# ChristophReich1996/Semantic_Pyramid_for_Image_Generation

Measured on AMD Instinct MI355X. Metric: images/sec full G+D train step, 256x256, bs/GPU=20, higher is better.
Workload: dtype bf16

## Files before the change

### include/sempyr.h

```cpp
#ifndef SEMPYR_H
#define SEMPYR_H
#include <stdint.h>

#ifdef __cplusplus
extern "C" {
#endif

#define SP_VERSION 1

typedef void* sp_stream_t;

enum sp_status { SP_OK = 0, SP_ERR_INVALID = -1, SP_ERR_LAUNCH = -2, SP_ERR_UNSUPPORTED = -3 };
enum sp_dtype { SP_F32 = 0, SP_BF16 = 1, SP_F8 = 2 ,
                SP_F16 = 3 ,
                SP_F8_F16 = 4  };
enum sp_act { SP_ACT_NONE = 0, SP_ACT_LRELU = 1, SP_ACT_RELU = 2, SP_ACT_TANH = 3 };

int sp_version(void);

enum { SP_TUNE_CONV_TALL = 0, SP_TUNE_IGEMM_DMA = 1, SP_TUNE_WGRAD_ROWS = 2, SP_TUNE_DETERMINISTIC = 3,
       SP_TUNE_SPLITK_TARGET = 4, SP_TUNE_SPLITK_MINSTEPS = 5, SP_TUNE_CONV1X1_DIRECT = 6, SP_TUNE_CONV_SHORT = 7,
       SP_TUNE_WGRAD9_BLOCKS = 8, SP_TUNE_WGRAD_BLOCKS = 9, SP_TUNE_WGRAD_MINSTEPS = 10, SP_TUNE_WGRAD_SMALL_M = 11,
       SP_TUNE_WGRAD_K1_TILE64 = 12, SP_TUNE_WGRAD_ROWS_THIN = 13, SP_TUNE_WGRAD_ROWS_BLOCKS = 14, SP_TUNE_WGRAD_ROWS_SLABS = 15,
       SP_TUNE_CONV_STAGGER = 16, SP_TUNE_CONV1X1_SPLITK = 17, SP_TUNE_WGRAD1X1 = 18, SP_TUNE_CONV_CIN8 = 19, SP_TUNE_CONV_THINCO = 20, SP_TUNE_CONV_PP = 21, SP_TUNE_CONV_PP_PRIO = 22, SP_TUNE_WGRAD_PP = 23, SP_TUNE_BN_ITERS = 24, SP_TUNE_IGEMM_TILE = 25, SP_TUNE_CONV_PPW = 26, SP_TUNE_LINEAR_KS = 27, SP_TUNE_CONV_PP_SPLIT = 28, SP_TUNE_COUNT = 29 };
int sp_set_tuning(int32_t key, int32_t value);
const char* sp_last_error_string(void);
const char* sp_last_route(void);

typedef struct sp_conv_params {
    const void* x;
    const void* w;
    const float* bias;
    void* y;
    const void* res1;
    const void* res2;
    const void* mask_src;
    float mask_neg_slope;
    int32_t n, h, w_, cin_p, cout, ldy, ksize, act, dtype;
    void* workspace;
    int64_t workspace_bytes;
    int32_t pool2;
    int32_t in_up2;
    const float* x_scale;
    const float* w_scale;
    void* y8;
    const float* y8_inv_scale;
    float* y8_amax;
    const float* img_scale;
    int32_t img_split;
    int32_t reserved_;
    int64_t split_pix_;
    const void* tail_w;
    const float* tail_bias;
    void* tail_y;
    int32_t tail_cout, tail_act, tail_ld, reserved2_;
    uint32_t* pool_idx;
    int32_t* split_sync;
} sp_conv_params;
#define SP_CONV_SPLIT_SYNC_BYTES 8192
int sp_conv2d_igemm(const sp_conv_params* p, sp_stream_t stream);
int sp_conv2d_workspace(int32_t n, int32_t h, int32_t w_, int32_t cin_p, int32_t cout, int32_t ksize, int32_t dtype,
                        int64_t* bytes_out);
int sp_conv2d_route(const sp_conv_params* p, const char** route);

int sp_conv2d_wgrad(const void* x, const void* dy, float* dw, int32_t n, int32_t h, int32_t w_,
                    int32_t cin_p, int32_t cout, int32_t ld_dy, int32_t ksize, int32_t dtype,
                    sp_stream_t stream);

int sp_conv2d_wgrad_fused(const void* x, const void* dy, float* dw, float* dbias, const void* w_packed, float* dot,
                          float* workspace, int64_t workspace_floats, int32_t n, int32_t h, int32_t w_, int32_t cin_p,
                          int32_t cout, int32_t ld_dy, int32_t ksize, int32_t dtype, sp_stream_t stream);
int sp_conv2d_wgrad_accum(const void* x, const void* dy, float* dw, float* dbias, float* workspace, int64_t workspace_floats,
                          int32_t n, int32_t h, int32_t w_, int32_t cin_p, int32_t cout, int32_t ld_dy, int32_t ksize,
                          int32_t dtype, sp_stream_t stream);
int sp_conv2d_wgrad_accum_pooled(const void* x, const void* dy, float* dw, float* dbias, float* workspace, int64_t workspace_floats,
                                 int32_t n, int32_t h, int32_t w_, int32_t cin_p, int32_t cout, int32_t ld_dy, int32_t ksize,
                                 int32_t dtype, sp_stream_t stream);
// ... 227 lines not shown
```

### semantic_pyramid_for_image_generation_amd/_lib.py

```python
from __future__ import annotations

import ctypes
import os
import re
from typing import Dict, List, Tuple

_HERE = os.path.dirname(os.path.abspath(__file__))
HEADER = os.path.join(os.path.dirname(_HERE), "include", "sempyr.h")
LIB_PATH = os.environ.get("SEMPYR_LIB") or os.path.join(_HERE, "libsempyr.so")

SP_F32, SP_BF16, SP_F8, SP_F16, SP_F8_F16 = 0, 1, 2, 3, 4
ACT_NONE, ACT_LRELU, ACT_RELU, ACT_TANH = 0, 1, 2, 3

TUNE_KEYS = {"SP_CONV_TALL": 0, "SP_IGEMM_DMA": 1, "SP_WGRAD_ROWS": 2, "SP_DETERMINISTIC": 3, "SP_SPLITK_TARGET": 4,
             "SP_SPLITK_MINSTEPS": 5, "SP_CONV1X1_DIRECT": 6, "SP_CONV_SHORT": 7, "SP_WGRAD9_BLOCKS": 8, "SP_WGRAD_BLOCKS": 9,
             "SP_WGRAD_MINSTEPS": 10, "SP_WGRAD_SMALL_M": 11, "SP_WGRAD_K1_TILE64": 12, "SP_WGRAD_ROWS_THIN": 13,
             "SP_WGRAD_ROWS_BLOCKS": 14, "SP_WGRAD_ROWS_SLABS": 15, "SP_CONV_STAGGER": 16, "SP_CONV1X1_SPLITK": 17, "SP_WGRAD1X1": 18, "SP_CONV_CIN8": 19, "SP_CONV_THINCO": 20,
             "SP_CONV_PP": 21, "SP_CONV_PP_PRIO": 22, "SP_WGRAD_PP": 23, "SP_BN_ITERS": 24, "SP_IGEMM_TILE": 25, "SP_CONV_PPW": 26, "SP_LINEAR_KS": 27, "SP_CONV_PP_SPLIT": 28}


SP_CONV_SPLIT_SYNC_BYTES = 8192


class SpConvParams(ctypes.Structure):
    _fields_ = [("x", ctypes.c_void_p), ("w", ctypes.c_void_p), ("bias", ctypes.c_void_p), ("y", ctypes.c_void_p),
                ("res1", ctypes.c_void_p), ("res2", ctypes.c_void_p), ("mask_src", ctypes.c_void_p),
                ("mask_neg_slope", ctypes.c_float),
                ("n", ctypes.c_int32), ("h", ctypes.c_int32), ("w_", ctypes.c_int32), ("cin_p", ctypes.c_int32),
                ("cout", ctypes.c_int32), ("ldy", ctypes.c_int32), ("ksize", ctypes.c_int32), ("act", ctypes.c_int32),
                ("dtype", ctypes.c_int32), ("workspace", ctypes.c_void_p), ("workspace_bytes", ctypes.c_int64),
                ("pool2", ctypes.c_int32), ("in_up2", ctypes.c_int32),
                ("x_scale", ctypes.c_void_p), ("w_scale", ctypes.c_void_p), ("y8", ctypes.c_void_p),
                ("y8_inv_scale", ctypes.c_void_p), ("y8_amax", ctypes.c_void_p),
                ("img_scale", ctypes.c_void_p), ("img_split", ctypes.c_int32), ("reserved_", ctypes.c_int32),
                ("split_pix_", ctypes.c_int64),
                ("tail_w", ctypes.c_void_p), ("tail_bias", ctypes.c_void_p), ("tail_y", ctypes.c_void_p),
                ("tail_cout", ctypes.c_int32), ("tail_act", ctypes.c_int32), ("tail_ld", ctypes.c_int32), ("reserved2_", ctypes.c_int32),
                ("pool_idx", ctypes.c_void_p), ("split_sync", ctypes.c_void_p)]


class SpConvGeneralParams(ctypes.Structure):
    _fields_ = [("struct_bytes", ctypes.c_int32), ("dtype", ctypes.c_int32),
                ("x", ctypes.c_void_p), ("w", ctypes.c_void_p), ("bias", ctypes.c_void_p), ("y", ctypes.c_void_p),
                ("n", ctypes.c_int32), ("h", ctypes.c_int32), ("w_", ctypes.c_int32), ("cin_p", ctypes.c_int32),
                ("ldx", ctypes.c_int32), ("cout", ctypes.c_int32), ("ldy", ctypes.c_int32), ("kh", ctypes.c_int32),
                ("kw", ctypes.c_int32), ("stride_h", ctypes.c_int32), ("stride_w", ctypes.c_int32), ("pad_h", ctypes.c_int32),
                ("pad_w", ctypes.c_int32), ("act", ctypes.c_int32)]

    def __init__(self, **kw):
        super().__init__(struct_bytes=ctypes.sizeof(SpConvGeneralParams), **kw)


class SpSnLayer(ctypes.Structure):
    _fields_ = [("w", ctypes.c_void_p), ("u", ctypes.c_void_p), ("v", ctypes.c_void_p),
                ("scratch_off", ctypes.c_int64), ("part_off", ctypes.c_int64), ("fwd_off", ctypes.c_int64),
                ("dgrad_off", ctypes.c_int64),
                ("rows", ctypes.c_int32), ("cols", ctypes.c_int32), ("cin", ctypes.c_int32), ("taps", ctypes.c_int32),
                ("cin_p", ctypes.c_int32), ("cout_p", ctypes.c_int32), ("kind", ctypes.c_int32),
                ("pack_block0", ctypes.c_int32)]


class SpSnBwdLayer(ctypes.Structure):
    _fields_ = [("w", ctypes.c_void_p), ("dw_off", ctypes.c_int64), ("dot_off", ctypes.c_int64),
                ("scratch_off", ctypes.c_int64), ("grad_off", ctypes.c_int64),
                ("rows", ctypes.c_int32), ("cols", ctypes.c_int32), ("cin", ctypes.c_int32), ("taps", ctypes.c_int32),
                ("cin_p", ctypes.c_int32), ("plain", ctypes.c_int32), ("db_off", ctypes.c_int32),
                ("bias_off", ctypes.c_int32)]


class SpRecLevel(ctypes.Structure):
    _fields_ = [("real", ctypes.c_void_p), ("fake", ctypes.c_void_p), ("mask", ctypes.c_void_p), ("dfake", ctypes.c_void_p),
# ... 72 lines not shown
```

### semantic_pyramid_for_image_generation_amd/csrc/attention.hip

```cpp
#include "common.h"

namespace {


template <typename T, int TQ>
__global__ __launch_bounds__(256) void attn_fwd_kernel(const T* __restrict__ q, const T* __restrict__ k, const T* __restrict__ v,
                                                       T* __restrict__ o, float* __restrict__ lse, int N, int NK, int D, int DV) {
    extern __shared__ __attribute__((aligned(16))) float sm[];
    float* ks = sm;
    float* qs = ks + NK * (D + 1);
    float* S = qs + TQ * D;
    float* vs = S + TQ * NK;
    const int tid = threadIdx.x, lane = tid & 63, wave = tid >> 6;
    const int b = blockIdx.y, q0 = blockIdx.x * TQ;
    const T* kb = k + (long)b * NK * D;
    const T* vb = v + (long)b * NK * DV;
    const T* qb = q + ((long)b * N + q0) * D;
    for (int e = tid; e < NK * D; e += 256) ks[(e / D) * (D + 1) + e % D] = Elem<T>::ld(kb + e);
    for (int e = tid; e < TQ * D; e += 256) qs[e] = (q0 + e / D < N) ? Elem<T>::ld(qb + e) : 0.f;
    __syncthreads();
    for (int j = tid; j < NK; j += 256) {
        const float* kr = ks + j * (D + 1);
        for (int qi = 0; qi < TQ; ++qi) {
            float s = 0.f;
// ... 417 lines not shown
            }
        }
    }
    {
        f32x4_t acc[4][4];
        const int ndb = D / 16;
#pragma unroll
        for (int a = 0; a < 4; ++a)
#pragma unroll
            for (int db = 0; db < 4; ++db) acc[a][db] = f32x4_t{0.f, 0.f, 0.f, 0.f};
#pragma unroll
        for (int t2 = 0; t2 < AB_QB / 32; ++t2) {
            uint4 sb[4];
#pragma unroll
            for (int a = 0; a < 4; ++a) {
                const int kf = wave + 4 * a;
                sb[a] = tr_pair(dSsm + (t2 * 32 + rowsel) * PP + colsel + (kf < nf ? kf : 0) * 32, 16 * PP);
            }
#pragma unroll
            for (int db = 0; db < 4; ++db)
                if (db < ndb) {
                    const uint4 qa = tr_pair(Qsm + (t2 * 32 + rowsel) * PK + colsel + db * 32, 16 * PK);
#pragma unroll
                    for (int a = 0; a < 4; ++a)
                        acc[a][db] = __builtin_amdgcn_mfma_f32_16x16x32_bf16(__builtin_bit_cast(bf16x8_t, qa), __builtin_bit_cast(bf16x8_t, sb[a]), acc[a][db], 0, 0, 0);
                }
        }
#pragma unroll
        for (int a = 0; a < 4; ++a) {
            const int kf = wave + 4 * a;
            if (kf < nf) {
                float* dst = dk_slab + ((long)b * NK + kf * 16 + i16) * D + g * 4;
#pragma unroll
                for (int db = 0; db < 4; ++db)
                    if (db < ndb) *reinterpret_cast<float4*>(dst + db * 16) = make_float4(acc[a][db][0], acc[a][db][1], acc[a][db][2], acc[a][db][3]);
            }
        }
    }
}

template <typename T>
__global__ void attn_reduce_kernel(const float* __restrict__ src, int nslabs, long n, T* __restrict__ dst) {
    for (long i = (long)blockIdx.x * 256 + threadIdx.x; i < n / 4; i += (long)gridDim.x * 256) {
        float4 a = reinterpret_cast<const float4*>(src)[i];
        for (int s = 1; s < nslabs; ++s) {
            const float4 t = reinterpret_cast<const float4*>(src + (long)s * n)[i];
            a.x += t.x; a.y += t.y; a.z += t.z; a.w += t.w;
        }
        const float o[4] = {a.x, a.y, a.z, a.w};
        Elem<T>::st4(dst + i * 4, o);
    }
}

template <typename T>
__global__ void cast_f32_kernel(const float* __restrict__ src, T* __restrict__ dst, long n) {
    for (long i = (long)blockIdx.x * 256 + threadIdx.x; i < n; i += (long)gridDim.x * 256) Elem<T>::st(dst + i, src[i]);
}

template <typename T, int TQ>
int launch_attn_tq(bool fwd, const void* q, const void* k, const void* v, void* o_or_dq, const void* dout, float* lse, float* dk,
                   float* dv, int B, int N, int NK, int D, int DV, hipStream_t s) {
    const int lds_f = (NK * (D + 1) + TQ * D + TQ * NK + 32 * DV) * 4;
    const int lds_b = (NK * (D + 1) + TQ * D + TQ * DV + TQ * NK + TQ * 4 + 32 * (NK + 1)) * 4;
    dim3 grid(sp_div_up(N, TQ), B);
    if (fwd) {
        if (const int rc = sp_lds_limit<attn_fwd_kernel<T, TQ>>(lds_f)) return rc;
        hipLaunchKernelGGL((attn_fwd_kernel<T, TQ>), grid, dim3(256), lds_f, s, (const T*)q, (const T*)k, (const T*)v, (T*)o_or_dq, lse, N, NK, D, DV);
    } else {
        if (const int rc = sp_lds_limit<attn_bwd_kernel<T, TQ>>(lds_b)) return rc;
        hipLaunchKernelGGL((attn_bwd_kernel<T, TQ>), grid, dim3(256), lds_b, s, (const T*)q, (const T*)k, (const T*)v, (const T*)dout, lse,
                           (T*)o_or_dq, dk, dv, N, NK, D, DV);
    }
    SP_LAUNCH_CHECK();
    return SP_OK;
}

inline int attn_valu_tq(int NK, int D, int DV) {
    const long lds_b32 = (long)(NK * (D + 1) + 32 * D + 32 * DV + 32 * NK + 32 * 4 + 32 * (NK + 1)) * 4;
    return lds_b32 <= 160 * 1024 ? 32 : 16;
}
inline bool attn_bwd_mfma_ok(int dtype, int nk, int d, int dv) {
    return dtype == SP_BF16 && (d == 32 || d == 64) && dv % 32 == 0 && dv <= 256 && nk % 32 == 0;
}
template <typename T>
int launch_attn(bool fwd, const void* q, const void* k, const void* v, void* o_or_dq, const void* dout, float* lse, float* dk,
                float* dv, int B, int N, int NK, int D, int DV, hipStream_t s) {
    if (attn_valu_tq(NK, D, DV) == 32) return launch_attn_tq<T, 32>(fwd, q, k, v, o_or_dq, dout, lse, dk, dv, B, N, NK, D, DV, s);
    return launch_attn_tq<T, 16>(fwd, q, k, v, o_or_dq, dout, lse, dk, dv, B, N, NK, D, DV, s);
}

}

extern "C" int sp_attention_fwd(const void* q, const void* k, const void* v, void* o, float* lse, int32_t batch, int32_t n,
                                int32_t nk, int32_t d, int32_t dv, int32_t dtype, sp_stream_t stream) {
    SP_CHECK_ARG(q && k && v && o && lse, "sp_attention_fwd: null pointer");
    SP_CHECK_ARG(nk > 0 && nk <= 256 && d > 0 && d <= 64 && dv > 0 && dv <= 256, "sp_attention_fwd: unsupported extents nk=%d d=%d dv=%d", nk, d, dv);
    hipStream_t s = reinterpret_cast<hipStream_t>(stream);
    if (dtype == SP_BF16 && d % 32 == 0 && dv % 16 == 0 && dv <= 256 && nk % 32 == 0) {
        const int lds = nk * (dv * 2 + 32);
        if (const int rc = sp_lds_limit<attn_fwd_mfma_kernel>(lds)) return rc;
        hipLaunchKernelGGL(attn_fwd_mfma_kernel, dim3(sp_div_up(n, 64), batch), dim3(256), lds, s, (const bf16*)q, (const bf16*)k, (const bf16*)v,
                           (bf16*)o, lse, n, nk, d, dv);
        SP_LAUNCH_CHECK();
        return SP_OK;
    }
    return dtype == SP_F32 ? launch_attn<float>(true, q, k, v, o, nullptr, lse, nullptr, nullptr, batch, n, nk, d, dv, s)
                           : launch_attn<bf16>(true, q, k, v, o, nullptr, lse, nullptr, nullptr, batch, n, nk, d, dv, s);
}

extern "C" int sp_attention_bwd(const void* q, const void* k, const void* v, const void* dout, const float* lse, void* dq,
                                float* dk_f32, float* dv_f32, void* dk, void* dv_out, int32_t batch, int32_t n, int32_t nk,
                                int32_t d, int32_t dv, int32_t dtype, sp_stream_t stream) {
    SP_CHECK_ARG(q && k && v && dout && lse && dq && dk_f32 && dv_f32 && dk && dv_out, "sp_attention_bwd: null pointer");
    SP_CHECK_ARG(nk > 0 && nk <= 256 && d > 0 && d <= 64 && dv > 0 && dv <= 256, "sp_attention_bwd: unsupported extents nk=%d d=%d dv=%d", nk, d, dv);
    hipStream_t s = reinterpret_cast<hipStream_t>(stream);
    const long nkd = (long)batch * nk * d, nkv = (long)batch * nk * dv;
    if (attn_bwd_mfma_ok(dtype, nk, d, dv)) {
        const int nqb = sp_div_up(n, AB_QB);
        const int lds = nk * (d * 2 + 32) + AB_QB * (d * 2 + 32) + AB_QB * (dv * 2 + 32) + 2 * AB_QB * (nk * 2 + 32);
        if (const int rc = sp_lds_limit<attn_bwd_mfma_kernel>(lds)) return rc;
        hipLaunchKernelGGL(attn_bwd_mfma_kernel, dim3(nqb, batch), dim3(256), lds, s, (const bf16*)q, (const bf16*)k,
                           (const bf16*)v, (const bf16*)dout, lse, (bf16*)dq, dk_f32, dv_f32, n, nk, d, dv);
        hipLaunchKernelGGL(attn_reduce_kernel<bf16>, dim3(sp_div_up(nkd / 4, 256)), dim3(256), 0, s, dk_f32, nqb, nkd, (bf16*)dk);
        hipLaunchKernelGGL(attn_reduce_kernel<bf16>, dim3(sp_div_up(nkv / 4, 256)), dim3(256), 0, s, dv_f32, nqb, nkv, (bf16*)dv_out);
        SP_LAUNCH_CHECK();
        return SP_OK;
    }
    SP_CHECK_ARG(nkd % 4 == 0 && nkv % 4 == 0, "sp_attention_bwd: batch*nk*d and batch*nk*dv must be multiples of 4");
    const int nqb = sp_div_up(n, attn_valu_tq(nk, d, dv));
    int rc = dtype == SP_F32 ? launch_attn<float>(false, q, k, v, dq, dout, const_cast<float*>(lse), dk_f32, dv_f32, batch, n, nk, d, dv, s)
                             : launch_attn<bf16>(false, q, k, v, dq, dout, const_cast<float*>(lse), dk_f32, dv_f32, batch, n, nk, d, dv, s);
    if (rc != SP_OK) return rc;
    if (dtype == SP_F32) {
        hipLaunchKernelGGL(attn_reduce_kernel<float>, dim3(sp_div_up(nkd / 4, 256)), dim3(256), 0, s, dk_f32, nqb, nkd, (float*)dk);
        hipLaunchKernelGGL(attn_reduce_kernel<float>, dim3(sp_div_up(nkv / 4, 256)), dim3(256), 0, s, dv_f32, nqb, nkv, (float*)dv_out);
    } else {
        hipLaunchKernelGGL(attn_reduce_kernel<bf16>, dim3(sp_div_up(nkd / 4, 256)), dim3(256), 0, s, dk_f32, nqb, nkd, (bf16*)dk);
        hipLaunchKernelGGL(attn_reduce_kernel<bf16>, dim3(sp_div_up(nkv / 4, 256)), dim3(256), 0, s, dv_f32, nqb, nkv, (bf16*)dv_out);
    }
    SP_LAUNCH_CHECK();
    return SP_OK;
}

extern "C" int sp_attention_bwd_slabs(int32_t n, int32_t nk, int32_t d, int32_t dv, int32_t dtype, int64_t* slabs_out) {
    SP_CHECK_ARG(slabs_out && n > 0 && nk > 0 && d > 0 && dv > 0, "sp_attention_bwd_slabs: bad args");
    *slabs_out = attn_bwd_mfma_ok(dtype, nk, d, dv) ? sp_div_up(n, AB_QB) : sp_div_up(n, attn_valu_tq(nk, d, dv));
    return SP_OK;
}
```

### semantic_pyramid_for_image_generation_amd/ops.py

```python
from __future__ import annotations

import ctypes
import os
from typing import List, Optional, Sequence

import torch

from . import _lib as L
from .config import CFG

ACT_NONE, ACT_LRELU, ACT_RELU, ACT_TANH = L.ACT_NONE, L.ACT_LRELU, L.ACT_RELU, L.ACT_TANH

_STATE = {"dtype": torch.float32, "vgg_fp8": int(CFG.vgg_fp8), "loss_scale": float(CFG.f16_loss_scale)}


def set_compute_dtype(dtype: torch.dtype) -> None:
    if dtype not in (torch.float32, torch.bfloat16, torch.float16):
        raise ValueError("compute dtype must be torch.float32, torch.bfloat16 or torch.float16")
    _STATE["dtype"] = dtype


def is_16bit(dtype: torch.dtype) -> bool:
    return dtype in (torch.bfloat16, torch.float16)

# ... 531 lines not shown
                break
            i = short[0]
            a, b = merged[i]
            cand = [j for j, (c, d) in enumerate(merged) if j != i and (d == a or c == b)]
            if not cand:
                break
            j = min(cand, key=lambda k: abs(k - i))
            c, d = merged[j]
            merged[max(i, j)] = (min(a, c), max(b, d))
            del merged[min(i, j)]
        if tail is not None:
            merged.append(tail)
        out = []
        for a, b in merged:
            while a < b:
                e = min(b, a + bucket_floats)
                if b - e < min_floats and b - a >= min_floats:
                    e = b
                out.append((a, e))
                a = e
        return out


def packed_layer(module, training: bool, dtype, device) -> PackedLayer:
    bank = getattr(module, "_sn_bank", None)
    if bank is not None and bank.current is not None and bank.current.dtype == dtype:
        return bank.current.layers[module._sn_slot]
    solo = getattr(module, "_sn_solo", None)
    if solo is None:
        saved = (getattr(module, "_sn_bank", None), getattr(module, "_sn_slot", None))
        solo = SpectralNormBank([(module, module._sn_kind, True)])
        module._sn_solo = solo
        module._sn_bank, module._sn_slot = saved
    call = solo.begin(training, dtype, device)
    solo.current = None
    return call.layers[0]


KERNEL_PROBE = None
PROBE_NET = ["sn"]


def _probed(family: str, flops: float, fn, shape=None) -> None:
    e0, e1 = torch.cuda.Event(enable_timing=True), torch.cuda.Event(enable_timing=True)
    e0.record()
    fn()
    e1.record()
    route = L.lib().sp_last_route().decode()
    KERNEL_PROBE.append((e0, e1, flops, family, None, route, shape, PROBE_NET[0]))


TUNE_CONV_TALL, TUNE_IGEMM_DMA, TUNE_WGRAD_ROWS, TUNE_DETERMINISTIC = 0, 1, 2, 3
TUNE_CONV1X1_SPLITK, TUNE_WGRAD1X1, TUNE_CONV_CIN8, TUNE_CONV_THINCO = 17, 18, 19, 20
_POOL2_BWD_FUSED = CFG.pool2_bwd_fused


def set_tuning(key: int, value: int) -> None:
    L.call("sp_set_tuning", key, value)
    _CONV_WS_CACHE.clear()
    _WS_CACHE.clear()
    _POOLED_WGRAD_CACHE.clear()
    _LIN_WS_CACHE.clear()


def conv_launch(x, w_ptr: int, bias, y, res1, res2, mask_src, slope: float, n, h, w, cin_p, cout, ldy, ksize, act,
                dtype, pool2: bool = False, in_up2: bool = False, family: str = "fwd", img_scale: int = 0, img_split: int = 0,
                k_real: Optional[int] = None, pool_idx: Optional[torch.Tensor] = None) -> None:
    if KERNEL_PROBE is not None:
        _probed(family, 2.0 * n * h * w * (k_real if k_real is not None else cin_p) * cout * ksize * ksize,
                lambda: _conv_launch(x, w_ptr, bias, y, res1, res2, mask_src, slope, n, h, w, cin_p, cout, ldy, ksize, act, dtype, pool2, in_up2,
                                     img_scale, img_split, pool_idx),
                (ksize, cin_p, cout, h, w, n))
        return
    _conv_launch(x, w_ptr, bias, y, res1, res2, mask_src, slope, n, h, w, cin_p, cout, ldy, ksize, act, dtype, pool2, in_up2, img_scale, img_split,
                 pool_idx)


def conv_pool2_ok(h: int, w: int, cout: int, ksize: int) -> bool:
    return ksize == 3 and cout > 32 and cout % 16 == 0 and h % 8 == 0 and w % 32 == 0


def conv_pool_idx_ok(n: int, h: int, w: int, cin_p: int, cout: int, dtype) -> bool:
    esz = 4 if dtype == torch.float32 else 2
    return (conv_pool2_ok(h, w, cout, 3) and cout % 16 == 0 and n * h * w * cin_p * esz < (1 << 30) and cout * 9 * cin_p * esz < (1 << 30))


_SPLIT_SYNC = {}


def _split_sync(device) -> torch.Tensor:
    key = (torch.device(device).index, torch.cuda.current_stream(device).cuda_stream)
    t = _SPLIT_SYNC.get(key)
    if t is None:
        t = _SPLIT_SYNC[key] = torch.zeros(L.SP_CONV_SPLIT_SYNC_BYTES // 4, dtype=torch.int32, device=device)
    return t


def _conv_launch(x, w_ptr: int, bias, y, res1, res2, mask_src, slope: float, n, h, w, cin_p, cout, ldy, ksize, act,
                 dtype, pool2: bool = False, in_up2: bool = False, img_scale: int = 0, img_split: int = 0, pool_idx=None) -> None:
    p = L.SpConvParams()
    if pool_idx is not None:
        p.pool_idx = pool_idx.data_ptr()
    if img_scale:
        p.img_scale, p.img_split = img_scale, img_split
    p.x, p.w, p.bias, p.y = x.data_ptr(), w_ptr, (bias.data_ptr() if bias is not None else None), y.data_ptr()
    p.res1 = res1.data_ptr() if res1 is not None else None
# ... 1122 lines not shown
```

Before: 1369.

## Add persistent multi-tile attention forward and backward kernels sized to CU count

Adds attention kernels where each block walks several query tiles, so the V (and K) shared-memory staging is loaded once per block instead of once per 64-row tile. In the backward pass, dK/dV accumulate in registers across tiles and are written directly to bf16 when one block covers a batch; otherwise a fused pair-reduce kernel sums the per-block slabs. The tile count per block is chosen so that blocks times batch fits roughly one or two waves over 256 CUs, with a tuning key to force it. The cost is less parallelism per launch and longer-lived register accumulators, and the CU count is hard-coded.

```diff
diff --git a/include/sempyr.h b/include/sempyr.h
--- a/include/sempyr.h
+++ b/include/sempyr.h
@@ -22,7 +22,8 @@
        SP_TUNE_SPLITK_TARGET = 4, SP_TUNE_SPLITK_MINSTEPS = 5, SP_TUNE_CONV1X1_DIRECT = 6, SP_TUNE_CONV_SHORT = 7,
        SP_TUNE_WGRAD9_BLOCKS = 8, SP_TUNE_WGRAD_BLOCKS = 9, SP_TUNE_WGRAD_MINSTEPS = 10, SP_TUNE_WGRAD_SMALL_M = 11,
        SP_TUNE_WGRAD_K1_TILE64 = 12, SP_TUNE_WGRAD_ROWS_THIN = 13, SP_TUNE_WGRAD_ROWS_BLOCKS = 14, SP_TUNE_WGRAD_ROWS_SLABS = 15,
-       SP_TUNE_CONV_STAGGER = 16, SP_TUNE_CONV1X1_SPLITK = 17, SP_TUNE_WGRAD1X1 = 18, SP_TUNE_CONV_CIN8 = 19, SP_TUNE_CONV_THINCO = 20, SP_TUNE_CONV_PP = 21, SP_TUNE_CONV_PP_PRIO = 22, SP_TUNE_WGRAD_PP = 23, SP_TUNE_BN_ITERS = 24, SP_TUNE_IGEMM_TILE = 25, SP_TUNE_CONV_PPW = 26, SP_TUNE_LINEAR_KS = 27, SP_TUNE_CONV_PP_SPLIT = 28, SP_TUNE_COUNT = 29 };
+       SP_TUNE_CONV_STAGGER = 16, SP_TUNE_CONV1X1_SPLITK = 17, SP_TUNE_WGRAD1X1 = 18, SP_TUNE_CONV_CIN8 = 19, SP_TUNE_CONV_THINCO = 20, SP_TUNE_CONV_PP = 21, SP_TUNE_CONV_PP_PRIO = 22, SP_TUNE_WGRAD_PP = 23, SP_TUNE_BN_ITERS = 24, SP_TUNE_IGEMM_TILE = 25, SP_TUNE_CONV_PPW = 26, SP_TUNE_LINEAR_KS = 27, SP_TUNE_CONV_PP_SPLIT = 28, SP_TUNE_ATTN_TILES = 29,
+       SP_TUNE_COUNT = 30 };
 int sp_set_tuning(int32_t key, int32_t value);
 const char* sp_last_error_string(void);
 const char* sp_last_route(void);
diff --git a/profiles/attention_floor.py b/profiles/attention_floor.py
--- /dev/null
+++ b/profiles/attention_floor.py
@@ -0,0 +1,47 @@
+import re
+import sys
+
+N, NK, D, DV = 1024, 256, 32, 128
+HBM, PEAK = 4e12, 2.5e15
+ORDER = {"fwd": [40, 40, 20], "bwd": [40, 20, 20]}
+
+
+def floor_us(kind, b):
+    if kind == "fwd":
+        nbytes = b * (N * D + NK * D + NK * DV + N * DV) * 2 + b * N * 4
+        flops = 2 * b * N * NK * (D + DV)
+    else:
+        nbytes = b * (2 * N * D + 2 * NK * D + 2 * NK * DV + N * DV) * 2 + b * N * 4
+        flops = 2 * b * N * NK * (3 * D + 2 * DV)
+    return max(nbytes / HBM, flops / PEAK) * 1e6
+
+
+def launches(path):
+    out, seen = [], {"fwd": 0, "bwd": 0}
+    for line in open(path):
+        m = re.match(r"\s*[\d.]+\s+([\d.]+) gap\s+[\d.]+\s+(attn_\w+)", line)
+        if not m:
+            continue
+        us, name = float(m.group(1)), m.group(2)
+        if "reduce" in name:
+            out[-1][2] += us
+            continue
+        kind = "fwd" if "fwd" in name else "bwd"
+        out.append([kind, ORDER[kind][seen[kind]], us])
+        seen[kind] += 1
+    return out
+
+
+def main():
+    for path in sys.argv[1:]:
+        rows = launches(path)
+        total, fl = sum(r[2] for r in rows), sum(floor_us(r[0], r[1]) for r in rows)
+        print(path)
+        for kind, b, us in rows:
+            f = floor_us(kind, b)
+            print("  %s batch %2d: %6.1f us   floor %4.1f us   %4.1f x floor" % (kind, b, us, f, us / f))
+        print("  attention family: %.1f us per step, floor %.1f us (%.1f %% of the floor reached)" % (total, fl, 100 * fl / total))
+
+
+if __name__ == "__main__":
+    main()
diff --git a/profiles/pmc_by_kernel.py b/profiles/pmc_by_kernel.py
--- /dev/null
+++ b/profiles/pmc_by_kernel.py
@@ -0,0 +1,17 @@
+import collections
+import csv
+import re
+import sys
+
+agg = collections.defaultdict(list)
+for r in csv.DictReader(open(sys.argv[1])):
+    name = re.sub(r"\(anonymous namespace\)::", "", r["Kernel_Name"]).replace("void ", "").split("(")[0]
+    if "attn" not in name:
+        continue
+    agg[(name, r.get("Grid_Size", "?"), r["Counter_Name"])].append(float(r["Counter_Value"]))
+last = None
+for (name, grid, ctr), v in sorted(agg.items()):
+    if (name, grid) != last:
+        print("%s grid %s: %d dispatches" % (name, grid, len(v)))
+        last = (name, grid)
+    print("  %-28s %.6e" % (ctr, sum(v) / len(v)))
diff --git a/semantic_pyramid_for_image_generation_amd/_lib.py b/semantic_pyramid_for_image_generation_amd/_lib.py
--- a/semantic_pyramid_for_image_generation_amd/_lib.py
+++ b/semantic_pyramid_for_image_generation_amd/_lib.py
@@ -16,7 +16,8 @@
              "SP_SPLITK_MINSTEPS": 5, "SP_CONV1X1_DIRECT": 6, "SP_CONV_SHORT": 7, "SP_WGRAD9_BLOCKS": 8, "SP_WGRAD_BLOCKS": 9,
              "SP_WGRAD_MINSTEPS": 10, "SP_WGRAD_SMALL_M": 11, "SP_WGRAD_K1_TILE64": 12, "SP_WGRAD_ROWS_THIN": 13,
              "SP_WGRAD_ROWS_BLOCKS": 14, "SP_WGRAD_ROWS_SLABS": 15, "SP_CONV_STAGGER": 16, "SP_CONV1X1_SPLITK": 17, "SP_WGRAD1X1": 18, "SP_CONV_CIN8": 19, "SP_CONV_THINCO": 20,
-             "SP_CONV_PP": 21, "SP_CONV_PP_PRIO": 22, "SP_WGRAD_PP": 23, "SP_BN_ITERS": 24, "SP_IGEMM_TILE": 25, "SP_CONV_PPW": 26, "SP_LINEAR_KS": 27, "SP_CONV_PP_SPLIT": 28}
+             "SP_CONV_PP": 21, "SP_CONV_PP_PRIO": 22, "SP_WGRAD_PP": 23, "SP_BN_ITERS": 24, "SP_IGEMM_TILE": 25, "SP_CONV_PPW": 26, "SP_LINEAR_KS": 27, "SP_CONV_PP_SPLIT": 28,
+             "SP_ATTN_TILES": 29}
 
 
 SP_CONV_SPLIT_SYNC_BYTES = 8192
diff --git a/semantic_pyramid_for_image_generation_amd/csrc/attention.hip b/semantic_pyramid_for_image_generation_amd/csrc/attention.hip
--- a/semantic_pyramid_for_image_generation_amd/csrc/attention.hip
+++ b/semantic_pyramid_for_image_generation_amd/csrc/attention.hip
@@ -493,6 +493,401 @@
     }
 }
 
+constexpr int AT_CUS = 256;
+struct ChunkIt {
+    int row, c, dr, dc, cpr;
+    __device__ __forceinline__ ChunkIt(int tid, int cpr_) : cpr(cpr_) { row = tid / cpr; c = tid - row * cpr; dr = 256 / cpr; dc = 256 - dr * cpr; }
+    __device__ __forceinline__ void next() { row += dr; c += dc; if (c >= cpr) { c -= cpr; ++row; } }
+};
+template <int NR>
+__device__ __forceinline__ void at_load(uint4 (&r)[NR], const bf16* __restrict__ src, int ld, int rows_valid, int cpr, int tid) {
+    ChunkIt it(tid, cpr);
+#pragma unroll
+    for (int i = 0; i < NR; ++i) {
+        r[i] = make_uint4(0, 0, 0, 0);
+        if (it.row < rows_valid) r[i] = *reinterpret_cast<const uint4*>(src + (long)it.row * ld + it.c * 8);
+        it.next();
+    }
+}
+template <int NR>
+__device__ __forceinline__ void at_store(const uint4 (&r)[NR], char* sm, int pitch, int rows, int cpr, int tid) {
+    ChunkIt it(tid, cpr);
+#pragma unroll
+    for (int i = 0; i < NR; ++i) {
+        if (it.row < rows) *reinterpret_cast<uint4*>(sm + it.row * pitch + it.c * 16) = r[i];
+        it.next();
+    }
+}
+template <int CPR, int NR>
+__device__ __forceinline__ void at_load_c(uint4 (&r)[NR], const bf16* __restrict__ src, int rows_valid, int tid) {
+#pragma unroll
+    for (int i = 0; i < NR; ++i) {
+        const int e = tid + i * 256, row = e / CPR, c = e % CPR;
+        r[i] = make_uint4(0, 0, 0, 0);
+        if (row < rows_valid) r[i] = *reinterpret_cast<const uint4*>(src + (long)row * (CPR * 8) + c * 8);
+    }
+}
+template <int CPR, int NR>
+__device__ __forceinline__ void at_store_c(const uint4 (&r)[NR], char* sm, int pitch, int rows, int tid) {
+#pragma unroll
+    for (int i = 0; i < NR; ++i) {
+        const int e = tid + i * 256, row = e / CPR, c = e % CPR;
+        if (row < rows) *reinterpret_cast<uint4*>(sm + row * pitch + c * 16) = r[i];
+    }
+}
+
+__global__ __launch_bounds__(256) void attn_fwd_tiles_kernel(const bf16* __restrict__ q, const bf16* __restrict__ k,
+                                                             const bf16* __restrict__ v, bf16* __restrict__ o, float* __restrict__ lse,
+                                                             int N, int NK, int D, int DV, int tiles) {
+    extern __shared__ __attribute__((aligned(16))) char vsm[];
+    const int PV = DV * 2 + 32;
+    const int tid = threadIdx.x, lane = tid & 63, wave = tid >> 6;
+    const int b = blockIdx.y;
+    const int ntiles = (N + 63) / 64;
+    const int t0 = blockIdx.x * tiles, t1 = min(t0 + tiles, ntiles);
+    const bf16* kb = k + (long)b * NK * D;
+    const bf16* vb = v + (long)b * NK * DV;
+    const int i16 = lane & 15, g = lane >> 4;
+    const int nf = NK / 16, ncb = DV / 16;
+    uint4 qv0, qv1;
+    {
+        const bf16* qp = q + ((long)b * N + min(t0 * 64 + wave * 16 + i16, N - 1)) * D + g * 8;
+        qv0 = *reinterpret_cast<const uint4*>(qp);
+        qv1 = D > 32 ? *reinterpret_cast<const uint4*>(qp + 32) : qv0;
+    }
+    {
+        const int cpr = DV / 8, half = NK / 2;
+        uint4 r[16];
+        at_load(r, vb, DV, half, cpr, tid);
+        at_store(r, vsm, PV, half, cpr, tid);
+        at_load(r, vb + (long)half * DV, DV, half, cpr, tid);
+        at_store(r, vsm + half * PV, PV, half, cpr, tid);
+    }
+    for (int t = t0; t < t1; ++t) {
+        const int q0 = t * 64 + wave * 16;
+        f32x4_t sfr[AM_NKMAX / 16];
+#pragma unroll
+        for (int f = 0; f < AM_NKMAX / 16; ++f) sfr[f] = f32x4_t{0.f, 0.f, 0.f, 0.f};
+#pragma unroll
+        for (int dd = 0; dd < 2; ++dd) {
+            if (dd * 32 < D) {
+                const uint4 qd = dd == 0 ? qv0 : qv1;
+#pragma unroll
+                for (int f = 0; f < AM_NKMAX / 16; ++f) {
+                    if (f < nf) {
+                        const uint4 kv = *reinterpret_cast<const uint4*>(kb + (long)(f * 16 + i16) * D + dd * 32 + g * 8);
+                        sfr[f] = __builtin_amdgcn_mfma_f32_16x16x32_bf16(__builtin_bit_cast(bf16x8_t, kv), __builtin_bit_cast(bf16x8_t, qd), sfr[f], 0, 0, 0);
+                    }
+                }
+            }
+        }
+        if (t + 1 < t1) {
+            const bf16* qp = q + ((long)b * N + min(q0 + 64 + i16, N - 1)) * D + g * 8;
+            qv0 = *reinterpret_cast<const uint4*>(qp);
+            if (D > 32) qv1 = *reinterpret_cast<const uint4*>(qp + 32);
+        }
+        float m = -INFINITY;
+#pragma unroll
+        for (int f = 0; f < AM_NKMAX / 16; ++f)
+            if (f < nf) m = fmaxf(fmaxf(fmaxf(m, sfr[f][0]), fmaxf(sfr[f][1], sfr[f][2])), sfr[f][3]);
+        m = fmaxf(m, __shfl_xor(m, 16, 64));
+        m = fmaxf(m, __shfl_xor(m, 32, 64));
+        float sum = 0.f;
+#pragma unroll
+        for (int f = 0; f < AM_NKMAX / 16; ++f)
+            if (f < nf) {
+#pragma unroll
+                for (int r = 0; r < 4; ++r) { const float e = __expf(sfr[f][r] - m); sfr[f][r] = e; sum += e; }
+            }
+        sum += __shfl_xor(sum, 16, 64);
+        sum += __shfl_xor(sum, 32, 64);
+        const float inv = 1.f / sum;
+        if (g == 0 && q0 + i16 < N) lse[(long)b * N + q0 + i16] = m + __logf(sum);
+        if (t == t0) __syncthreads();
+        f32x4_t oacc[16];
+#pragma unroll
+        for (int cb = 0; cb < 16; ++cb) oacc[cb] = f32x4_t{0.f, 0.f, 0.f, 0.f};
+#pragma unroll
+        for (int tk = 0; tk < AM_NKMAX / 32; ++tk) {
+            if (tk * 32 < NK) {
+                uint4 pb;
+                pb.x = f32x2_to_bf16x2(sfr[2 * tk][0] * inv, sfr[2 * tk][1] * inv);
+                pb.y = f32x2_to_bf16x2(sfr[2 * tk][2] * inv, sfr[2 * tk][3] * inv);
+                pb.z = f32x2_to_bf16x2(sfr[2 * tk + 1][0] * inv, sfr[2 * tk + 1][1] * inv);
+                pb.w = f32x2_to_bf16x2(sfr[2 * tk + 1][2] * inv, sfr[2 * tk + 1][3] * inv);
+                const char* vrow = vsm + (tk * 32 + g * 4 + (i16 >> 2)) * PV + (i16 & 3) * 8;
+#pragma unroll
+                for (int cb = 0; cb < 16; ++cb) {
+                    if (cb < ncb) {
+                        const uint4 va = tr_pair(vrow + cb * 32, 16 * PV);
+                        oacc[cb] = __builtin_amdgcn_mfma_f32_16x16x32_bf16(__builtin_bit_cast(bf16x8_t, va), __builtin_bit_cast(bf16x8_t, pb), oacc[cb], 0, 0, 0);
+                    }
+                }
+            }
+        }
+        if (q0 + i16 < N) {
+            bf16* op = o + ((long)b * N + q0 + i16) * DV + g * 4;
+#pragma unroll
+            for (int cb = 0; cb < 16; ++cb)
+                if (cb < ncb) {
+                    const float t4[4] = {oacc[cb][0], oacc[cb][1], oacc[cb][2], oacc[cb][3]};
+                    Elem<bf16>::st4(op + cb * 16, t4);
+                }
+        }
+    }
+}
+
+template <int D, int DV>
+__global__ __launch_bounds__(256) void attn_bwd_tiles_kernel(const bf16* __restrict__ q, const bf16* __restrict__ k,
+                                                             const bf16* __restrict__ v, const bf16* __restrict__ dout,
+                                                             const float* __restrict__ lse, bf16* __restrict__ dq,
+                                                             float* __restrict__ dk32, float* __restrict__ dv32,
+                                                             bf16* __restrict__ dk_out, bf16* __restrict__ dv_out,
+                                                             int N, int NK, int tiles) {
+    extern __shared__ __attribute__((aligned(16))) char bsm[];
+    constexpr int PK = D * 2 + 32, PDO = DV * 2 + 32;
+    const int PP = NK * 2 + 32;
+    char* Ksm = bsm;
+    char* Qsm = Ksm + NK * PK;
+    char* dOsm = Qsm + AB_QB * PK;
+    char* Psm = dOsm + AB_QB * PDO;
+    char* dSsm = Psm + AB_QB * PP;
+    constexpr int PVL = DV * 2 + 16;
+    const int tid = threadIdx.x, lane = tid & 63, wave = tid >> 6;
+    const int b = blockIdx.y;
+    const int ntiles = (N + AB_QB - 1) / AB_QB;
+    const int t0 = blockIdx.x * tiles, t1 = min(t0 + tiles, ntiles);
+    const bool direct = gridDim.x == 1;
+    const bf16* kb = k + (long)b * NK * D;
+    const bf16* vb = v + (long)b * NK * DV;
+    constexpr int cpr = D / 8, cpo = DV / 8, ndb = D / 16, ncb = DV / 16;
+    const int i16 = lane & 15, g = lane >> 4;
+    const int ql = wave * 16 + i16;
+    const int nf = NK / 16;
+    const int rowsel = g * 4 + (i16 >> 2), colsel = (i16 & 3) * 8;
+    uint4 nq[D / 32], ndo[DV / 32];
+    float nl;
+    at_load_c<cpr>(nq, q + ((long)b * N + t0 * AB_QB) * D, min(AB_QB, N - t0 * AB_QB), tid);
+    at_load_c<cpo>(ndo, dout + ((long)b * N + t0 * AB_QB) * DV, min(AB_QB, N - t0 * AB_QB), tid);
+    nl = t0 * AB_QB + ql < N ? lse[(long)b * N + t0 * AB_QB + ql] : 0.f;
+    {
+        uint4 r[8];
+        at_load_c<cpr>(r, kb, NK, tid);
+        at_store_c<cpr>(r, Ksm, PK, NK, tid);
+    }
+    f32x4_t dva[4][ncb], dka[4][ndb];
+#pragma unroll
+    for (int a = 0; a < 4; ++a) {
+#pragma unroll
+        for (int cb = 0; cb < ncb; ++cb) dva[a][cb] = f32x4_t{0.f, 0.f, 0.f, 0.f};
+#pragma unroll
+        for (int db = 0; db < ndb; ++db) dka[a][db] = f32x4_t{0.f, 0.f, 0.f, 0.f};
+    }
+    for (int t = t0; t < t1; ++t) {
+        const int qb0 = t * AB_QB;
+        const bool q_ok = qb0 + ql < N;
+        const float l = nl;
+        int tl = tid;
+        asm volatile("" : "+v"(tl));
+        at_store_c<cpr>(nq, Qsm, PK, AB_QB, tl);
+        at_store_c<cpo>(ndo, dOsm, PDO, AB_QB, tl);
+        {
+            uint4 r[8];
+            at_load_c<cpo>(r, vb, NK / 2, tl);
+            at_store_c<cpo>(r, Psm, PVL, NK / 2, tl);
+            at_load_c<cpo>(r, vb + (long)(NK / 2) * DV, NK / 2, tl);
+            at_store_c<cpo>(r, Psm + (NK / 2) * PVL, PVL, NK / 2, tl);
+        }
+        __syncthreads();
+        f32x4_t pfr[AM_NKMAX / 16], dpf[AM_NKMAX / 16];
+#pragma unroll
+        for (int f = 0; f < AM_NKMAX / 16; ++f) { pfr[f] = f32x4_t{0.f, 0.f, 0.f, 0.f}; dpf[f] = f32x4_t{0.f, 0.f, 0.f, 0.f}; }
+#pragma unroll
+        for (int d0 = 0; d0 < D; d0 += 32) {
+            const uint4 qv = *reinterpret_cast<const uint4*>(Qsm + ql * PK + (d0 + g * 8) * 2);
+#pragma unroll
+            for (int f = 0; f < AM_NKMAX / 16; ++f)
+                if (f < nf) {
+                    const uint4 kv = *reinterpret_cast<const uint4*>(Ksm + (f * 16 + i16) * PK + (d0 + g * 8) * 2);
+                    pfr[f] = __builtin_amdgcn_mfma_f32_16x16x32_bf16(__builtin_bit_cast(bf16x8_t, kv), __builtin_bit_cast(bf16x8_t, qv), pfr[f], 0, 0, 0);
+                }
+        }
+#pragma unroll
+        for (int f = 0; f < AM_NKMAX / 16; ++f)
+#pragma unroll
+            for (int r = 0; r < 4; ++r) { float x = pfr[f][r]; asm volatile("" : "+v"(x)); pfr[f][r] = x; }
+#pragma unroll
+        for (int c0 = 0; c0 < DV; c0 += 32) {
+            const uint4 dov = *reinterpret_cast<const uint4*>(dOsm + ql * PDO + (c0 + g * 8) * 2);
+#pragma unroll
+            for (int f = 0; f < AM_NKMAX / 16; ++f)
+                if (f < nf) {
+                    const uint4 vv = *reinterpret_cast<const uint4*>(Psm + (f * 16 + i16) * PVL + (c0 + g * 8) * 2);
+                    dpf[f] = __builtin_amdgcn_mfma_f32_16x16x32_bf16(__builtin_bit_cast(bf16x8_t, vv), __builtin_bit_cast(bf16x8_t, dov), dpf[f], 0, 0, 0);
+                }
+        }
+        float drow = 0.f;
+#pragma unroll
+        for (int f = 0; f < AM_NKMAX / 16; ++f)
+            if (f < nf) {
+#pragma unroll
+                for (int r = 0; r < 4; ++r) {
+                    const float pv = q_ok ? __expf(pfr[f][r] - l) : 0.f;
+                    pfr[f][r] = pv;
+                    drow += pv * dpf[f][r];
+                }
+            }
+        drow += __shfl_xor(drow, 16, 64);
+        drow += __shfl_xor(drow, 32, 64);
+#pragma unroll
+        for (int f = 0; f < AM_NKMAX / 16; ++f)
+            if (f < nf) {
+#pragma unroll
+                for (int r = 0; r < 4; ++r) dpf[f][r] = pfr[f][r] * (dpf[f][r] - drow);
+            }
+        {
+            f32x4_t dqa[ndb];
+#pragma unroll
+            for (int db = 0; db < ndb; ++db) dqa[db] = f32x4_t{0.f, 0.f, 0.f, 0.f};
+#pragma unroll
+            for (int tk = 0; tk < AM_NKMAX / 32; ++tk)
+                if (tk * 32 < NK) {
+                    const uint4 sb = pack8(dpf[2 * tk], dpf[2 * tk + 1]);
+                    const char* krow = Ksm + (tk * 32 + rowsel) * PK + colsel;
+#pragma unroll
+                    for (int db = 0; db < ndb; ++db)
+                        if (db < ndb) {
+                            const uint4 ka = tr_pair(krow + db * 32, 16 * PK);
+                            dqa[db] = __builtin_amdgcn_mfma_f32_16x16x32_bf16(__builtin_bit_cast(bf16x8_t, ka), __builtin_bit_cast(bf16x8_t, sb), dqa[db], 0, 0, 0);
+                        }
+                }
+            if (q_ok) {
+                bf16* qp = dq + ((long)b * N + qb0 + ql) * D + g * 4;
+#pragma unroll
+                for (int db = 0; db < ndb; ++db)
+                    if (db < ndb) {
+                        const float t4[4] = {dqa[db][0], dqa[db][1], dqa[db][2], dqa[db][3]};
+                        Elem<bf16>::st4(qp + db * 16, t4);
+                    }
+            }
+        }
+        __syncthreads();
+#pragma unroll
+        for (int f = 0; f < AM_NKMAX / 16; ++f)
+            if (f < nf) {
+                uint2 pw, sw;
+                pw.x = f32x2_to_bf16x2(pfr[f][0], pfr[f][1]);
+                pw.y = f32x2_to_bf16x2(pfr[f][2], pfr[f][3]);
+                sw.x = f32x2_to_bf16x2(dpf[f][0], dpf[f][1]);
+                sw.y = f32x2_to_bf16x2(dpf[f][2], dpf[f][3]);
+                *reinterpret_cast<uint2*>(Psm + ql * PP + (f * 16 + g * 4) * 2) = pw;
+                *reinterpret_cast<uint2*>(dSsm + ql * PP + (f * 16 + g * 4) * 2) = sw;
+            }
+        __syncthreads();
+        if (t + 1 < t1) {
+            const int nb0 = qb0 + AB_QB;
+            at_load_c<cpr>(nq, q + ((long)b * N + nb0) * D, min(AB_QB, N - nb0), tl);
+            at_load_c<cpo>(ndo, dout + ((long)b * N + nb0) * DV, min(AB_QB, N - nb0), tl);
+            nl = nb0 + ql < N ? lse[(long)b * N + nb0 + ql] : 0.f;
+        }
+#pragma unroll
+        for (int a = 0; a < 4; ++a) {
+#pragma unroll
+            for (int cb = 0; cb < ncb; ++cb)
+#pragma unroll
+                for (int r = 0; r < 4; ++r) { float x = dva[a][cb][r]; asm volatile("" : "+a"(x)); dva[a][cb][r] = x; }
+#pragma unroll
+            for (int db = 0; db < ndb; ++db)
+#pragma unroll
+                for (int r = 0; r < 4; ++r) { float x = dka[a][db][r]; asm volatile("" : "+a"(x)); dka[a][db][r] = x; }
+        }
+#pragma unroll
+        for (int t2 = 0; t2 < AB_QB / 32; ++t2) {
+            uint4 pb[4];
+#pragma unroll
+            for (int a = 0; a < 4; ++a) {
+                const int kf = wave + 4 * a;
+                pb[a] = tr_pair(Psm + (t2 * 32 + rowsel) * PP + colsel + (kf < nf ? kf : 0) * 32, 16 * PP);
+            }
+#pragma unroll
+            for (int cb = 0; cb < ncb; ++cb)
+                if (cb < ncb) {
+                    const uint4 da = tr_pair(dOsm + (t2 * 32 + rowsel) * PDO + colsel + cb * 32, 16 * PDO);
+#pragma unroll
+                    for (int a = 0; a < 4; ++a)
+                        dva[a][cb] = __builtin_amdgcn_mfma_f32_16x16x32_bf16(__builtin_bit_cast(bf16x8_t, da), __builtin_bit_cast(bf16x8_t, pb[a]), dva[a][cb], 0, 0, 0);
+                }
+        }
+#pragma unroll
+        for (int t2 = 0; t2 < AB_QB / 32; ++t2) {
+            uint4 sb[4];
+#pragma unroll
+            for (int a = 0; a < 4; ++a) {
+                const int kf = wave + 4 * a;
+                sb[a] = tr_pair(dSsm + (t2 * 32 + rowsel) * PP + colsel + (kf < nf ? kf : 0) * 32, 16 * PP);
+            }
+#pragma unroll
+            for (int db = 0; db < ndb; ++db)
+                if (db < ndb) {
+                    const uint4 qa = tr_pair(Qsm + (t2 * 32 + rowsel) * PK + colsel + db * 32, 16 * PK);
+#pragma unroll
+                    for (int a = 0; a < 4; ++a)
+                        dka[a][db] = __builtin_amdgcn_mfma_f32_16x16x32_bf16(__builtin_bit_cast(bf16x8_t, qa), __builtin_bit_cast(bf16x8_t, sb[a]), dka[a][db], 0, 0, 0);
+                }
+        }
+        if (t + 1 < t1) __syncthreads();
+    }
+#pragma unroll
+    for (int a = 0; a < 4; ++a) {
+        const int kf = wave + 4 * a;
+        if (kf < nf) {
+            const long row = (long)b * NK + kf * 16 + i16;
+            if (direct) {
+                bf16* dvp = dv_out + row * DV + g * 4;
+                bf16* dkp = dk_out + row * D + g * 4;
+#pragma unroll
+                for (int cb = 0; cb < ncb; ++cb)
+                    if (cb < ncb) {
+                        const float t4[4] = {dva[a][cb][0], dva[a][cb][1], dva[a][cb][2], dva[a][cb][3]};
+                        Elem<bf16>::st4(dvp + cb * 16, t4);
+                    }
+#pragma unroll
+                for (int db = 0; db < ndb; ++db)
+                    if (db < ndb) {
+                        const float t4[4] = {dka[a][db][0], dka[a][db][1], dka[a][db][2], dka[a][db][3]};
+                        Elem<bf16>::st4(dkp + db * 16, t4);
+                    }
+            } else {
+                float* dvp = dv32 + ((long)blockIdx.x * gridDim.y * NK + row) * DV + g * 4;
+                float* dkp = dk32 + ((long)blockIdx.x * gridDim.y * NK + row) * D + g * 4;
+#pragma unroll
+                for (int cb = 0; cb < ncb; ++cb)
+                    if (cb < ncb) *reinterpret_cast<float4*>(dvp + cb * 16) = make_float4(dva[a][cb][0], dva[a][cb][1], dva[a][cb][2], dva[a][cb][3]);
+#pragma unroll
+                for (int db = 0; db < ndb; ++db)
+                    if (db < ndb) *reinterpret_cast<float4*>(dkp + db * 16) = make_float4(dka[a][db][0], dka[a][db][1], dka[a][db][2], dka[a][db][3]);
+            }
+        }
+    }
+}
+
+template <typename T>
+__global__ void attn_reduce_pair_kernel(const float* __restrict__ dk32, const float* __restrict__ dv32, int nslabs, long nkd, long nkv,
+                                        T* __restrict__ dk, T* __restrict__ dv) {
+    const long i = (long)blockIdx.x * 256 + threadIdx.x;
+    if (i >= (nkd + nkv) / 4) return;
+    const bool isk = i < nkd / 4;
+    const float* src = isk ? dk32 : dv32;
+    const long n = isk ? nkd : nkv, e = isk ? i : i - nkd / 4;
+    float4 a = reinterpret_cast<const float4*>(src)[e];
+    for (int s = 1; s < nslabs; ++s) {
+        const float4 t = reinterpret_cast<const float4*>(src + (long)s * n)[e];
+        a.x += t.x; a.y += t.y; a.z += t.z; a.w += t.w;
+    }
+    const float o[4] = {a.x, a.y, a.z, a.w};
+    Elem<T>::st4((isk ? dk : dv) + e * 4, o);
+}
+
 template <typename T>
 __global__ void cast_f32_kernel(const float* __restrict__ src, T* __restrict__ dst, long n) {
     for (long i = (long)blockIdx.x * 256 + threadIdx.x; i < n; i += (long)gridDim.x * 256) Elem<T>::st(dst + i, src[i]);
@@ -523,6 +918,21 @@
 inline bool attn_bwd_mfma_ok(int dtype, int nk, int d, int dv) {
     return dtype == SP_BF16 && (d == 32 || d == 64) && dv % 32 == 0 && dv <= 256 && nk % 32 == 0;
 }
+inline bool attn_fwd_mfma_ok(int dtype, int nk, int d, int dv) {
+    return dtype == SP_BF16 && d % 32 == 0 && dv % 16 == 0 && dv <= 256 && nk % 32 == 0;
+}
+inline bool attn_bwd_tiles_ok(int dtype, int nk, int d, int dv) {
+    return attn_bwd_mfma_ok(dtype, nk, d, dv) && dv <= 128 && nk * (dv * 2 + 16) <= 2 * AB_QB * (nk * 2 + 32);
+}
+inline int attn_tiles(int batch, int n, int slots) {
+    const int ntiles = sp_div_up(n, AB_QB);
+    const int forced = sp_tune(SP_TUNE_ATTN_TILES, -1);
+    if (forced == 0) return 0;
+    if (forced > 0) return forced < ntiles ? forced : ntiles;
+    int t = 1;
+    while (t < ntiles && (long)sp_div_up(ntiles, t) * batch > slots) ++t;
+    return t;
+}
 template <typename T>
 int launch_attn(bool fwd, const void* q, const void* k, const void* v, void* o_or_dq, const void* dout, float* lse, float* dk,
                 float* dv, int B, int N, int NK, int D, int DV, hipStream_t s) {
@@ -537,8 +947,15 @@
     SP_CHECK_ARG(q && k && v && o && lse, "sp_attention_fwd: null pointer");
     SP_CHECK_ARG(nk > 0 && nk <= 256 && d > 0 && d <= 64 && dv > 0 && dv <= 256, "sp_attention_fwd: unsupported extents nk=%d d=%d dv=%d", nk, d, dv);
     hipStream_t s = reinterpret_cast<hipStream_t>(stream);
-    if (dtype == SP_BF16 && d % 32 == 0 && dv % 16 == 0 && dv <= 256 && nk % 32 == 0) {
+    if (attn_fwd_mfma_ok(dtype, nk, d, dv)) {
         const int lds = nk * (dv * 2 + 32);
+        if (const int tiles = attn_tiles(batch, n, 2 * AT_CUS)) {
+            if (const int rc = sp_lds_limit<attn_fwd_tiles_kernel>(lds)) return rc;
+            hipLaunchKernelGGL(attn_fwd_tiles_kernel, dim3(sp_div_up(sp_div_up(n, 64), tiles), batch), dim3(256), lds, s, (const bf16*)q,
+                               (const bf16*)k, (const bf16*)v, (bf16*)o, lse, n, nk, d, dv, tiles);
+            SP_LAUNCH_CHECK();
+            return SP_OK;
+        }
         if (const int rc = sp_lds_limit<attn_fwd_mfma_kernel>(lds)) return rc;
         hipLaunchKernelGGL(attn_fwd_mfma_kernel, dim3(sp_div_up(n, 64), batch), dim3(256), lds, s, (const bf16*)q, (const bf16*)k, (const bf16*)v,
                            (bf16*)o, lse, n, nk, d, dv);
@@ -556,6 +973,25 @@
     SP_CHECK_ARG(nk > 0 && nk <= 256 && d > 0 && d <= 64 && dv > 0 && dv <= 256, "sp_attention_bwd: unsupported extents nk=%d d=%d dv=%d", nk, d, dv);
     hipStream_t s = reinterpret_cast<hipStream_t>(stream);
     const long nkd = (long)batch * nk * d, nkv = (long)batch * nk * dv;
+    const int tiles = attn_bwd_tiles_ok(dtype, nk, d, dv) ? attn_tiles(batch, n, AT_CUS) : 0;
+    if (tiles > 0) {
+        const int nblk = sp_div_up(sp_div_up(n, AB_QB), tiles);
+        const int lds = nk * (d * 2 + 32) + AB_QB * (d * 2 + 32) + AB_QB * (dv * 2 + 32) + 2 * AB_QB * (nk * 2 + 32);
+#define SP_ATTN_BWD_TILES(D_, DV_)                                                                                                       \
+    if (d == D_ && dv == DV_) {                                                                                                          \
+        if (const int rc = sp_lds_limit<attn_bwd_tiles_kernel<D_, DV_>>(lds)) return rc;                                                 \
+        hipLaunchKernelGGL((attn_bwd_tiles_kernel<D_, DV_>), dim3(nblk, batch), dim3(256), lds, s, (const bf16*)q, (const bf16*)k,       \
+                           (const bf16*)v, (const bf16*)dout, lse, (bf16*)dq, dk_f32, dv_f32, (bf16*)dk, (bf16*)dv_out, n, nk, tiles);   \
+    }
+        SP_ATTN_BWD_TILES(32, 32) SP_ATTN_BWD_TILES(32, 64) SP_ATTN_BWD_TILES(32, 96) SP_ATTN_BWD_TILES(32, 128)
+        SP_ATTN_BWD_TILES(64, 32) SP_ATTN_BWD_TILES(64, 64) SP_ATTN_BWD_TILES(64, 96) SP_ATTN_BWD_TILES(64, 128)
+#undef SP_ATTN_BWD_TILES
+        if (nblk > 1)
+            hipLaunchKernelGGL(attn_reduce_pair_kernel<bf16>, dim3(sp_div_up((nkd + nkv) / 4, 256)), dim3(256), 0, s, dk_f32, dv_f32, nblk, nkd,
+                               nkv, (bf16*)dk, (bf16*)dv_out);
+        SP_LAUNCH_CHECK();
+        return SP_OK;
+    }
     if (attn_bwd_mfma_ok(dtype, nk, d, dv)) {
         const int nqb = sp_div_up(n, AB_QB);
         const int lds = nk * (d * 2 + 32) + AB_QB * (d * 2 + 32) + AB_QB * (dv * 2 + 32) + 2 * AB_QB * (nk * 2 + 32);
diff --git a/semantic_pyramid_for_image_generation_amd/ops.py b/semantic_pyramid_for_image_generation_amd/ops.py
--- a/semantic_pyramid_for_image_generation_amd/ops.py
+++ b/semantic_pyramid_for_image_generation_amd/ops.py
@@ -607,6 +607,7 @@
 
 TUNE_CONV_TALL, TUNE_IGEMM_DMA, TUNE_WGRAD_ROWS, TUNE_DETERMINISTIC = 0, 1, 2, 3
 TUNE_CONV1X1_SPLITK, TUNE_WGRAD1X1, TUNE_CONV_CIN8, TUNE_CONV_THINCO = 17, 18, 19, 20
+TUNE_ATTN_TILES = 29
 _POOL2_BWD_FUSED = CFG.pool2_bwd_fused
 
 
```

Result: no change. 1382, median of 6 (+0.9%).
